# shayaanjamil-10xe/aimet

Measured on AMD Instinct MI355X. Metric: fake-quant Gelem/s (ResNet-50 W8A8 QuantSim forward QDQ; + compute_encodings wall-clock), higher is better.
Workload: dtype f32; 1 GPU; resnet50_w8a8_per_channel_fake_quant_fwd; launch=hipgraph, weight_qdq=one batched launch, global_batch=256, per_gpu_batch=256, act_quantizers=55, weight_quantizers=54, weight_channels=27560, parallelism=dp1, compute_encodings_scheme=tf_enhanced act per-tensor + tf_enhanced weight per-channel sym

## Files before the change

### aimet_amd/csrc/calib_plan.cpp

```cpp
#include <algorithm>
#include <cstring>
#include <mutex>
#include <vector>

#include "tq_internal.hpp"

using namespace aimet_amd;

struct aimet_calib_plan
{
    int device = 0;
    std::vector<aimet_tensor_quantizer*> aq, pq;
    int32_t aset[4] = {}, pset[4] = {};
    std::vector<StatsJob> jobs;
    uint64_t mm = 0, hb = 0;
    StatsJob* dj_fresh = nullptr;
    StatsJob* dj_cont  = nullptr;
    bool all_pdf       = false;
    ZeroJob* dz_act  = nullptr;
    int nz_act       = 0;
    int64_t most_act = 0;
    ResetJob* dr_act = nullptr;
    ZeroJob* dz_par  = nullptr;
    int nz_par       = 0;
    int64_t most_par = 0;
    ResetJob* dr_par = nullptr;
    ChannelJob* dch   = nullptr;
    uint64_t ch_blocks = 0;
    bool ch_hist      = false;
    TfeTable tfe_act {}, tfe_par {};
    bool has_tfe_act = false, has_tfe_par = false;
    void* pinned_act = nullptr;
    void* pinned_par = nullptr;
    size_t pinned_act_bytes = 0, pinned_par_bytes = 0;
    int busy_act = 0, busy_par = 0;
    void* dev_block = nullptr;
    hipEvent_t done = nullptr;
};

namespace
{

constexpr int kParamSearchPerCu = 2;

struct Packer
{
    std::vector<unsigned char> host;
    size_t add(const void* p, size_t bytes)
    {
        const size_t off = (host.size() + 255) & ~size_t(255);
        host.resize(off + bytes);
        if (bytes && p)
            std::memcpy(host.data() + off, p, bytes);
        return off;
    }
};

bool tfe_searched(const aimet_tensor_quantizer* q)
{
    return q->hist && q->scheme == AIMET_QUANTIZATION_TF_ENHANCED;
}

std::vector<TfeJob> tfe_jobs(const std::vector<aimet_tensor_quantizer*>& qs, int64_t* total)
{
    std::vector<TfeJob> jobs;
    int64_t t = 0;
    for (aimet_tensor_quantizer* q: qs)
        if (tfe_searched(q))
        {
            jobs.push_back(TfeJob {q->d.pdf_init, q->d.hist_min, q->d.bucket_size, q->d.pdf, nullptr, t});
            t += q->C;
        }
    *total = t;
    return jobs;
}

struct DeadPlan
{
    int device;
    void* dev_block;
    void* pinned_act;
    void* pinned_par;
    hipEvent_t done;
};
struct Graveyard
{
    std::mutex m;
    std::vector<DeadPlan> items;
};
Graveyard& graveyard()
{
    static Graveyard* g = new Graveyard();
    return *g;
}

void reap_dead_plans()
{
    std::vector<DeadPlan> ready;
    {
        Graveyard& g = graveyard();
        std::lock_guard<std::mutex> lock(g.m);
        for (size_t i = 0; i < g.items.size();)
            if (g.items[i].done == nullptr || hipEventQuery(g.items[i].done) == hipSuccess)
            {
                ready.push_back(g.items[i]);
// ... 10 lines not shown
        if (d.pinned_act)
            (void) hipHostFree(d.pinned_act);
        if (d.pinned_par)
            (void) hipHostFree(d.pinned_par);
        if (d.done)
            (void) hipEventDestroy(d.done);
    }
}

void destroy_plan(aimet_calib_plan* p)
{
    if (p == nullptr)
        return;
    if (p->dev_block || p->pinned_act || p->pinned_par || p->done)
    {
        Graveyard& g = graveyard();
        std::lock_guard<std::mutex> lock(g.m);
        g.items.push_back(DeadPlan {p->device, p->dev_block, p->pinned_act, p->pinned_par, p->done});
    }
    delete p;
}

hipStream_t upload_stream(int device)
{
    static std::mutex m;
    static std::vector<hipStream_t> streams(64, nullptr);
    AIMET_REQUIRE(device >= 0 && device < 64, "device id out of range");
    std::lock_guard<std::mutex> lock(m);
    if (streams[(size_t) device] == nullptr)
        AIMET_HIP_CHECK(hipStreamCreateWithFlags(&streams[(size_t) device], hipStreamNonBlocking));
    return streams[(size_t) device];
}

void adopt(aimet_encoding_request* r, void* pinned, size_t bytes, bool has_tfe, int* busy)
{
    if (r == nullptr)
        return;
    if (has_tfe)
    {
        r->pinned          = pinned;
        r->pinned_bytes    = bytes;
        r->pinned_borrowed = true;
    }
    r->busy = busy;
    ++*busy;
}

}

extern "C" {

int aimet_calib_plan_create(aimet_tensor_quantizer* const* act_qs, const float* const* act_x, const int64_t* act_n,
                            int64_t n_act, aimet_tensor_quantizer* const* par_qs, const float* const* par_x,
                            const int64_t* par_outer, const int64_t* par_C, const int64_t* par_K, int64_t n_par,
                            const int32_t* act_settings, const int32_t* par_settings, int64_t* elem_counts_dev,
                            aimet_calib_plan** out)
{
    aimet_calib_plan* p = nullptr;
    const int rc        = guarded([&] {
        AIMET_REQUIRE(out != nullptr && act_settings != nullptr && par_settings != nullptr, "null argument");
        AIMET_REQUIRE(n_act >= 0 && n_par >= 0, "negative quantizer count");
        AIMET_REQUIRE((n_act == 0 || (act_qs && act_x && act_n)) &&
                          (n_par == 0 || (par_qs && par_x && par_outer && par_C && par_K)),
                      "null argument");
        *out = nullptr;
        reap_dead_plans();
        p    = new aimet_calib_plan;
        std::copy(act_settings, act_settings + 4, p->aset);
        std::copy(par_settings, par_settings + 4, p->pset);
        p->aq.assign(act_qs, act_qs + n_act);
        p->pq.assign(par_qs, par_qs + n_par);
        AIMET_REQUIRE((n_act == 0 || act_qs[0] != nullptr) && (n_par == 0 || par_qs[0] != nullptr), "null quantizer");
        p->device = n_act ? act_qs[0]->device : (n_par ? par_qs[0]->device : 0);
        for (auto* q: p->pq)
            AIMET_REQUIRE(q != nullptr && q->device == p->device, "quantizers of one calibration share a device");
        if (elem_counts_dev)
            require_device_ptr(elem_counts_dev, "element counts");
        Packer pk;
        size_t o_fresh = 0, o_cont = 0, o_parts = 0, o_zact = 0, o_ract = 0;
        std::vector<int64_t> part_offs;
        if (n_act)
        {
            p->jobs = make_jobs(act_qs, act_x, act_n, nullptr, n_act);
            int64_t k = 0;
            p->all_pdf = true;
            for (int64_t i = 0; i < n_act; ++i)
            {
                StatsJob& j = p->jobs[(size_t) i];
                p->all_pdf  = p->all_pdf && j.hist && !j.ent;
                if (elem_counts_dev && j.hist)
                {
                    j.count_dev = elem_counts_dev + k;
                    j.count_out = elem_counts_dev + k;
                    ++k;
                }
            }
            stats_layout(p->jobs, &p->mm, &p->hb);
            o_parts = pk.add(nullptr, sizeof(float) * 2 * p->mm);
            std::vector<StatsJob> fresh = p->jobs;
            for (auto& j: fresh)
            {
                j.fresh = 1;
                j.seen  = 0;
            }
            for (auto& j: p->jobs)
                j.fresh = 0;
            o_fresh = pk.add(fresh.data(), sizeof(StatsJob) * fresh.size());
            o_cont  = pk.add(p->jobs.data(), sizeof(StatsJob) * p->jobs.size());
            std::vector<ZeroJob> z;
            std::vector<ResetJob> r;
            for (auto* q: p->aq)
                reset_ranges(q, false, z, r);
            for (const ZeroJob& zj: z)
                p->most_act = std::max(p->most_act, zj.bytes);
            p->nz_act = (int) z.size();
            o_zact    = pk.add(z.data(), sizeof(ZeroJob) * z.size());
            o_ract    = pk.add(r.data(), sizeof(ResetJob) * r.size());
        }
        size_t o_zpar = 0, o_rpar = 0, o_ch = 0;
        if (n_par)
        {
            std::vector<ChannelJob> cj;
            for (int64_t i = 0; i < n_par; ++i)
                cj.push_back(make_channel_job(par_qs[i], par_x[i], par_outer[i], par_C[i], par_K[i]));
            p->ch_blocks = channel_layout(cj, &p->ch_hist);
            o_ch         = pk.add(cj.data(), sizeof(ChannelJob) * cj.size());
            std::vector<ZeroJob> z;
            std::vector<ResetJob> r;
            for (auto* q: p->pq)
                reset_ranges(q, true, z, r);
            for (const ZeroJob& zj: z)
                p->most_par = std::max(p->most_par, zj.bytes);
            p->nz_par = (int) z.size();
            o_zpar    = pk.add(z.data(), sizeof(ZeroJob) * z.size());
            o_rpar    = pk.add(r.data(), sizeof(ResetJob) * r.size());
        }
        int64_t ta = 0, tp = 0;
        std::vector<TfeJob> ja = tfe_jobs(p->aq, &ta), jp = tfe_jobs(p->pq, &tp);
        DeviceGuard g(p->device);
        if (ta)
        {
            p->pinned_act_bytes = sizeof(aimet_tf_encoding) * (size_t) ta;
            AIMET_HIP_CHECK(hipHostMalloc(&p->pinned_act, p->pinned_act_bytes, hipHostMallocDefault));
            std::memset(p->pinned_act, 0, p->pinned_act_bytes);
        }
        if (tp)
        {
            p->pinned_par_bytes = sizeof(aimet_tf_encoding) * (size_t) tp;
            AIMET_HIP_CHECK(hipHostMalloc(&p->pinned_par, p->pinned_par_bytes, hipHostMallocDefault));
            std::memset(p->pinned_par, 0, p->pinned_par_bytes);
        }
        for (auto& j: ja)
            j.out = static_cast<aimet_tf_encoding*>(p->pinned_act) + j.start;
        for (auto& j: jp)
            j.out = static_cast<aimet_tf_encoding*>(p->pinned_par) + j.start;
        const int sa = ta ? tfe_splits(ta, p->aset[1] != 0) : 1, sp = tp ? tfe_splits(tp, p->pset[1] != 0) : 1;
        const size_t o_ja = pk.add(ja.data(), sizeof(TfeJob) * ja.size());
        const size_t o_jp = pk.add(jp.data(), sizeof(TfeJob) * jp.size());
        const size_t o_pa = sa > 1 ? pk.add(nullptr, sizeof(uint64_t) * 2 * ta * sa) : 0;
        const size_t o_ka = sa > 1 ? pk.add(nullptr, sizeof(unsigned) * ta) : 0;
        const size_t o_pp = sp > 1 ? pk.add(nullptr, sizeof(uint64_t) * 2 * tp * sp) : 0;
        const size_t o_kp = sp > 1 ? pk.add(nullptr, sizeof(unsigned) * tp) : 0;
        pk.add(nullptr, 0);
        if (pk.host.empty())
        {
            *out = p;
            p    = nullptr;
            return;
        }
        AIMET_HIP_CHECK(hipMalloc(&p->dev_block, pk.host.size()));
        char* base = static_cast<char*>(p->dev_block);
// ... 21 lines not shown
            p->dr_par = reinterpret_cast<ResetJob*>(base + o_rpar);
        }
        hipStream_t up = upload_stream(p->device);
        AIMET_HIP_CHECK(hipMemcpyAsync(p->dev_block, pk.host.data(), pk.host.size(), hipMemcpyHostToDevice, up));
        AIMET_HIP_CHECK(hipStreamSynchronize(up));
        AIMET_HIP_CHECK(hipEventCreateWithFlags(&p->done, hipEventDisableTiming));
        if (ta)
        {
            p->has_tfe_act = true;
            p->tfe_act     = TfeTable {ja[0], reinterpret_cast<const TfeJob*>(base + o_ja), (int) ja.size(), ta,
                                   sa > 1 ? reinterpret_cast<uint64_t*>(base + o_pa) : nullptr,
                                   sa > 1 ? reinterpret_cast<unsigned*>(base + o_ka) : nullptr};
        }
        if (tp)
        {
            p->has_tfe_par = true;
            p->tfe_par     = TfeTable {jp[0], reinterpret_cast<const TfeJob*>(base + o_jp), (int) jp.size(), tp,
                                   sp > 1 ? reinterpret_cast<uint64_t*>(base + o_pp) : nullptr,
                                   sp > 1 ? reinterpret_cast<unsigned*>(base + o_kp) : nullptr,
                                   n_act ? kParamSearchPerCu : 0};
        }
        *out = p;
        p    = nullptr;
    });
    if (p)
        destroy_plan(p);
    return rc;
}

int aimet_calib_plan_launch(aimet_calib_plan* p, int stages, int reset, void* main_stream, void* side_stream,
                            aimet_encoding_request** act_req, aimet_encoding_request** par_req)
{
    aimet_encoding_request *ra = nullptr, *rp = nullptr;
    const int rc = guarded([&] {
        AIMET_REQUIRE(p != nullptr && act_req != nullptr && par_req != nullptr, "null argument");
        AIMET_REQUIRE(stages >= 1 && stages <= 7 && (stages == 7 || stages == 1 || stages == 2 || stages == 4),
                      "stages: 7 (the whole batch on one device) or 1, 2, 4 (the sharded calibration's steps)");
        *act_req = *par_req = nullptr;
        const int64_t n_act = (int64_t) p->aq.size(), n_par = (int64_t) p->pq.size();
        if (n_act == 0 && n_par == 0)
            return;
        if ((stages & 4) && p->has_tfe_act)
            AIMET_REQUIRE(p->busy_act == 0, "calibration plan: the previous activation request is not finished");
        if ((stages & 1) && p->has_tfe_par)
            AIMET_REQUIRE(p->busy_par == 0, "calibration plan: the previous parameter request is not finished");
        DeviceGuard g(p->device);
        hipStream_t ms = as_stream(main_stream), ss = as_stream(side_stream);
        const bool first = (stages & 1) != 0;
        if (first && ss != ms && (n_par || (reset && n_act)))
            stream_join(ss, ms);
        auto rest = [&] {
            if (reset && n_act)
            {
                launch_zero_table(p->dz_act, p->nz_act, p->most_act, ss);
                launch_reset_table(p->dr_act, (int) n_act, ss);
                for (auto* q: p->aq)
                    mark_reset(q);
                if (ss != ms)
                    stream_join(ms, ss);
            }
            if (n_par)
            {
                if (reset)
                {
                    launch_zero_table(p->dz_par, p->nz_par, p->most_par, ss);
                    launch_reset_table(p->dr_par, (int) n_par, ss);
                    for (auto* q: p->pq)
                        mark_reset(q);
                }
                launch_channel_table(p->dch, (int) n_par, p->ch_blocks, p->ch_hist, ss);
                for (auto* q: p->pq)
                    q->stats_updated = true;
                encodings_launch(p->pq.data(), n_par, (uint32_t) p->pset[0], p->pset[1], p->pset[2], p->pset[3], ss, rp,
                                 nullptr, p->has_tfe_par ? &p->tfe_par : nullptr);
                adopt(rp, p->pinned_par, p->pinned_par_bytes, p->has_tfe_par, &p->busy_par);
            }
        };
        if (n_act)
        {
            int phases = 0;
            if (stages & 1)
                phases |= kPhaseMinmax | (stages == 7 ? kPhaseFoldMinmax : 0);
            if (stages & 2)
                phases |= (stages == 7 ? 0 : kPhaseFoldMinmax) | kPhaseHistogram;
            if (stages & 4)
                phases |= kPhaseFoldHistogram;
            bool seen = !reset;
            for (auto* q: p->aq)
                seen = seen && q->stats_updated;
            const bool walk = n_act > 64 || (p->all_pdf && seen);
            const StatsJob* dj = (first && reset) ? p->dj_fresh : p->dj_cont;
            if (first)
                launch_stats_table(dj, (int) n_act, p->mm, p->hb, walk, phases, ms, rest);
            else
                launch_stats_table(dj, (int) n_act, p->mm, p->hb, walk, phases, ms);
            if (first)
                for (auto* q: p->aq)
                    q->stats_updated = true;
        }
        else if (first)
            rest();
        if (stages & 4)
        {
            encodings_launch(p->aq.data(), n_act, (uint32_t) p->aset[0], p->aset[1], p->aset[2], p->aset[3], ms, ra,
                             nullptr, p->has_tfe_act ? &p->tfe_act : nullptr);
            adopt(ra, p->pinned_act, p->pinned_act_bytes, p->has_tfe_act, &p->busy_act);
        }
        if (first && n_par && ss != ms)
            stream_join(ms, ss);
        if (p->done)
            AIMET_HIP_CHECK(hipEventRecord(p->done, ms));
    });
    if (rc != AIMET_OK)
    {
        release_request_after_error(ra);
        release_request_after_error(rp);
        return rc;
    }
    *act_req = ra;
    *par_req = rp;
    return rc;
}

int aimet_calib_plan_destroy(aimet_calib_plan* p)
{
    return guarded([&] {
        if (p == nullptr)
            return;
        AIMET_REQUIRE(p->busy_act == 0 && p->busy_par == 0,
                      "calibration plan: finish (or discard) its requests before destroying it");
        destroy_plan(p);
    });
}

}
```

### aimet_amd/csrc/quantizer.cpp

```cpp
#include <algorithm>
#include <atomic>
#include <chrono>
#include <cstring>
#include <mutex>
#include <thread>
#include <vector>

#include "encodings.hpp"
#include "tq_internal.hpp"

using namespace aimet_amd;

struct Slab
{
    void* base   = nullptr;
    size_t bytes = 0;
    std::atomic<int64_t> refs {0};
};

namespace
{

size_t align256(size_t b)
{
// ... 956 lines not shown
    int64_t ent_total = 0;
    for (int64_t c: entC)
        ent_total += c;
    aimet_tf_encoding* mse_dst = nullptr;
    EntropyOut* ent_dst        = nullptr;
    if (req->mse_total + ent_total > 0)
    {
        const size_t mse_bytes = sizeof(aimet_tf_encoding) * (size_t) req->mse_total;
        req->pinned_dev = take_pinned(mse_bytes + sizeof(EntropyOut) * (size_t) ent_total, &req->pinned_dev_bytes);
        mse_dst         = req->mse_total ? static_cast<aimet_tf_encoding*>(req->pinned_dev) : nullptr;
        ent_dst = ent_total ? reinterpret_cast<EntropyOut*>(static_cast<char*>(req->pinned_dev) + mse_bytes) : nullptr;
    }
    launch_mse_search_many(mse.data(), mseC.data(), (int) mse.size(), b, sym != 0, strict != 0, unsign != 0, st,
                           mse_dst);
    launch_entropy_search_many(ent.data(), entC.data(), (int) ent.size(), sym != 0, strict != 0, unsign != 0, st,
                               ent_dst, b);
    if (tfe_total > 0 && table != nullptr)
    {
        AIMET_REQUIRE(table->total == tfe_total && table->n == (int) tfe.size(),
                      "calibration plan: the TF-Enhanced search table does not match the quantizers");
        launch_tfe_table(*table, b, sym != 0, strict != 0, unsign != 0, st);
    }
    else if (tfe_total > 0)
    {
        req->pinned = take_pinned(sizeof(aimet_tf_encoding) * (size_t) tfe_total, &req->pinned_bytes);
        launch_tfe_search_many_to(tfe.data(), req->tfe_Cs.data(), (int) tfe.size(), b, sym, strict, unsign,
                                  static_cast<aimet_tf_encoding*>(req->pinned), st, prep);
    }
    req->done = take_event();
    AIMET_HIP_CHECK(hipEventRecord(req->done, st));
    return req;
}

void aimet_amd::await_event(hipEvent_t e)
{
    const auto t0 = std::chrono::steady_clock::now();
    for (;;)
    {
        const hipError_t q = hipEventQuery(e);
        if (q == hipSuccess)
            return;
        if (q != hipErrorNotReady)
            AIMET_HIP_CHECK(q);
        const auto waited = std::chrono::steady_clock::now() - t0;
        if (waited > std::chrono::milliseconds(20))
            break;
        if (waited > std::chrono::microseconds(200))
            std::this_thread::sleep_for(std::chrono::microseconds(20));
    }
    AIMET_HIP_CHECK(hipEventSynchronize(e));
}

void aimet_amd::stream_join(hipStream_t waiter, hipStream_t from)
{
    hipEvent_t e = take_event();
    RequestPool& p = request_pool();
    try
    {
        AIMET_HIP_CHECK(hipEventRecord(e, from));
        AIMET_HIP_CHECK(hipStreamWaitEvent(waiter, e, 0));
    }
    catch (...)
    {
        std::lock_guard<std::mutex> lock(p.m);
        p.events.push_back(e);
        throw;
    }
    std::lock_guard<std::mutex> lock(p.m);
    p.events.push_back(e);
}

extern "C" {

int aimet_tq_get_encodings_launch(aimet_tensor_quantizer* const* qs, int64_t nq, uint32_t bw, int sym, int strict,
                                  int unsign, void* stream, aimet_encoding_request** req_out)
{
    aimet_encoding_request* req = nullptr;
    const int rc = guarded([&] {
        AIMET_REQUIRE(req_out != nullptr, "null argument");
        *req_out = nullptr;
        encodings_launch(qs, nq, bw, sym, strict, unsign, as_stream(stream), req);
    });
    if (rc != AIMET_OK)
// ... 70 lines not shown
        return rc;
    }
    *act_req = ra;
    *par_req = rp;
    return rc;
}

int aimet_tq_get_encodings_finish(aimet_encoding_request* req, aimet_tf_encoding* out, int* valid)
{
    const int rc = guarded([&] {
        AIMET_REQUIRE(req != nullptr, "request is null");
        const int64_t nq = (int64_t) req->qs.size();
        if (out == nullptr && valid == nullptr)
        {
            if (nq && req->done)
            {
                DeviceGuard g(req->device);
                AIMET_HIP_CHECK(hipEventSynchronize(req->done));
            }
            return;
        }
        int64_t total = 0;
        for (aimet_tensor_quantizer* q: req->qs)
            total += q->C;
        AIMET_REQUIRE(out != nullptr || total == 0, "out is null");
        if (total)
            std::memset(out, 0, sizeof(aimet_tf_encoding) * total);
        for (int64_t i = 0; i < nq; ++i)
            if (valid)
                valid[i] = req->qs[i]->stats_updated ? 1 : 0;
        if (nq == 0)
            return;
        DeviceGuard g(req->device);
        await_event(req->done);
        auto* tfe = static_cast<const aimet_tf_encoding*>(req->pinned);
        for (size_t k = 0, src = 0; k < req->tfe_Cs.size(); src += req->tfe_Cs[k], ++k)
            std::memcpy(out + req->tfe_offs[k], tfe + src, sizeof(aimet_tf_encoding) * req->tfe_Cs[k]);
        std::vector<int64_t> offs((size_t) nq);
        for (int64_t i = 0, o = 0; i < nq; o += req->qs[(size_t) i]->C, ++i)
            offs[(size_t) i] = o;
        std::vector<char> from_pinned((size_t) nq, 0);
        std::vector<const EntropyOut*> dev((size_t) nq, nullptr);
        {
            auto* m = static_cast<const aimet_tf_encoding*>(req->pinned_dev);
            for (int64_t i: req->mse_q)
            {
                const int64_t C = req->qs[(size_t) i]->C;
                std::memcpy(out + offs[(size_t) i], m, sizeof(aimet_tf_encoding) * C);
                m += C;
                from_pinned[(size_t) i] = 1;
            }
            auto* r = reinterpret_cast<const EntropyOut*>(static_cast<const char*>(req->pinned_dev) +
                                                          sizeof(aimet_tf_encoding) * (size_t) req->mse_total);
            for (int64_t i: req->ent_q)
            {
                const int64_t C = req->qs[(size_t) i]->C;
                aimet_tf_encoding* o = out + offs[(size_t) i];
                bool flagged = false;
                for (int64_t c = 0; c < C; ++c)
                {
                    o[c]    = aimet_tf_encoding {r[c].min, r[c].max, r[c].delta, r[c].offset, r[c].bw};
                    flagged = flagged || r[c].status == kEntHost;
                }
                dev[(size_t) i]         = r;
                from_pinned[(size_t) i] = flagged ? 0 : 1;
                r += C;
            }
// ... 105 lines not shown
```

### aimet_amd/csrc/stats.hip

```cpp
#include "entropy_core.hpp"
#include "tq_state.hpp"

#include <algorithm>
#include <cfloat>
#include <cstdlib>
#include <vector>

namespace aimet_amd
{

namespace
{

constexpr int kWaves      = kBlock / 64;
constexpr int kHistUnroll = 4;
constexpr int kHistGrid   = 2048;

__device__ __forceinline__ float wave_min(float v)
{
#pragma unroll
    for (int o = 32; o > 0; o >>= 1)
        v = fminf(v, __shfl_xor(v, o, 64));
    return v;
}
// ... 697 lines not shown
    }
}

__global__ __launch_bounds__(kBlock) void fold_minmax_many_kernel(const StatsJob* __restrict__ jobs)
{
    const StatsJob& J = jobs[blockIdx.x];
    if (J.ent)
    {
        float2 m = reinterpret_cast<const float2*>(J.d.minmax)[0];
        ent_fold_one(J.d, 0, -m.x, m.y);
    }
    else if (threadIdx.x == 0)
        fold_one(J.d, 0, !J.hist);
}

template <int BLOCK, int COLS>
__global__ __launch_bounds__(BLOCK) void histogram_many_kernel(const StatsJob* __restrict__ jobs, int njobs)
{
    const StatsJob& J = jobs[find_job(jobs, njobs, blockIdx.x, true)];
    if (!J.hist)
        return;
    if (J.ent)
    {
        if (J.d.active[0])
            histogram_part<BLOCK, true, COLS>(J.x, J.n, J.vec, blockIdx.x - J.h_block0, J.h_blocks, J.d);
    }
    else if (J.d.pdf_init[0])
        histogram_part<BLOCK, false, COLS>(J.x, J.n, J.vec, blockIdx.x - J.h_block0, J.h_blocks, J.d);
}

__global__ __launch_bounds__(kPdfSize) void fold_histogram_many_kernel(const StatsJob* __restrict__ jobs)
{
    const StatsJob& J = jobs[blockIdx.x];
    if (!J.hist)
        return;
    if (J.ent)
    {
        if (J.d.active[0])
            ent_fold_hist_one(J.d, 0);
    }
    else if (J.d.pdf_init[0])
        fold_hist_one(J.d, 0, J.count_dev ? *J.count_dev : J.count);
}

__device__ __forceinline__ int find_channel_job(const ChannelJob* __restrict__ jobs, int njobs, uint32_t b)
{
    return find_job_ballot(jobs, njobs, b, [](const ChannelJob& j) { return j.block0; });
}

__device__ __forceinline__ void channel_minmax(const ChannelJob& J, int64_t c, float& mn, float& mx)
{
    mn = INFINITY;
    mx = -INFINITY;
    for (int64_t o = 0; o < J.outer; ++o)
    {
        const float* row = J.x + (o * J.C + c) * J.K;
        if (J.vec)
        {
            const float4* r4 = reinterpret_cast<const float4*>(row);
            for (int64_t k = threadIdx.x; k < J.K / 4; k += kBlock)
                accum4(r4[k], mn, mx);
        }
        else
        {
            for (int64_t k = threadIdx.x; k < J.K; k += kBlock)
            {
                mn = fminf(mn, row[k]);
// ... 410 lines not shown
```

### aimet_amd/csrc/tfe_core.hpp

```cpp
#pragma once

#include <cfloat>
#include <cmath>

#if defined(__HIPCC__)
#define AIMET_HD __host__ __device__
#else
#define AIMET_HD
#endif

namespace aimet_amd
{
namespace tfe
{

constexpr int kBins        = 512;
constexpr float kGamma     = 3.0f;
constexpr float kMinRangeF = (float) 0.01;
constexpr int kAsymF       = 17;
constexpr int kAsymO       = 21;
constexpr int kSymF        = 101;
constexpr int kMaxCand     = kAsymF * kAsymO + 1;

template <class T>
// ... 301 lines not shown
    if constexpr (!split)
    {
        for (int k = 0; k < B.nnz; ++k)
        {
            if (k < kLo)
            {
                double d = B.cd_c[k] - loMid;
                satLo += B.pdf_c[k] * (d * d);
            }
            if (k >= kHi)
            {
                double d = B.cd_c[k] - hiMid;
                satHi += B.pdf_c[k] * (d * d);
            }
            if (k >= kLo && k < kHi)
            {
                float v   = B.cf_c[k];
                int q     = quant_code(v, delta, offset, rcp, thr);
                float deq = delta * (q + offset);
                double d  = (double) (v - deq);
                quant += B.pdf_c[k] * (d * d);
            }
        }
        double c = kGamma * (satLo + satHi) + quant;
        return smin(c, DBL_MAX);
    }
    satLo = sat_sum(B, 0, kLo, loMid);
    satHi = sat_sum(B, kHi, B.nnz, hiMid);
    quant = quant_sum(B, kLo, kHi, delta, offset, rcp, thr);
    double c = kGamma * (satLo + satHi) + quant;
    return smin(c, DBL_MAX);
}

struct Result
{
    double min, max, delta, offset;
};

AIMET_HD inline Result finish(const Setup& s, float bestDelta, int bestOffset)
{
    float lo = smax(bestDelta * bestOffset, -FLT_MAX);
    float hi = smin(bestDelta * (bestOffset + s.steps), FLT_MAX);
    return Result {lo, hi, bestDelta, (double) bestOffset};
}

}
}
```

### aimet_amd/csrc/tfe_search.hip

```cpp
#include "tfe_core.hpp"

#include <algorithm>
#include <cstdlib>
#include <cstring>
#include <mutex>
#include "tq_state.hpp"

#include <mutex>
#include <vector>

namespace aimet_amd
{
namespace
{

struct Best
{
    double cost;
    int idx;
    float delta;
    int offset;
};

__device__ __forceinline__ bool better(const Best& a, const Best& b)
{
    if (a.idx < 0)
        return false;
    if (b.idx < 0)
        return true;
    return (a.cost < b.cost) || (a.cost == b.cost && a.idx < b.idx);
}

template <int BLOCK, bool SYMFORM>
__global__ __launch_bounds__(BLOCK, BLOCK == 128 ? 5 : (BLOCK == 64 ? 2 : 7)) void tfe_search_kernel(
    TfeJob one, const TfeJob* __restrict__ jobs, int njobs, int64_t total, int bw, int sym, int strict, int unsign,
    int splits, uint64_t* __restrict__ part, unsigned* __restrict__ tickets)
{
    constexpr int kW = BLOCK / 64;
    __shared__ double pdf_c[tfe::kBins];
    __shared__ double cd_c[tfe::kBins];
    __shared__ float cf_c[tfe::kBins];
    __shared__ float cf[tfe::kBins];
    __shared__ short pos[tfe::kBins];
    __shared__ float fseq[tfe::kSymF + 8];
    __shared__ int first, last, nnz;
    __shared__ Best wbest[kW];
    if (threadIdx.x == 0)
    {
        if (sym)
            tfe::fseq_sym(fseq);
        else
            tfe::fseq_asym(fseq);
    }
    const int lane = threadIdx.x & 63;
    for (int64_t gs = blockIdx.x; gs < total * splits; gs += gridDim.x)
    {
        const int64_t g = gs / splits;
        const int sp    = (int) (gs - g * splits);
        TfeJob j = one;
        if (jobs)
        {
            int lo = 0, hi = njobs - 1;
            while (lo < hi)
            {
                int mid = (lo + hi + 1) >> 1;
                if (jobs[mid].start <= g)
                    lo = mid;
                else
                    hi = mid - 1;
            }
            j = jobs[lo];
        }
        const int64_t c = g - j.start;
        if (!j.pdf_init[c])
        {
            if (threadIdx.x == 0 && sp == 0)
            {
                int isteps = (int) (float) (ldexp(1.0, bw) - 1);
                aimet_tf_encoding e;
                e.delta    = (1.0 - (-1.0)) / isteps;
                e.offset   = floor(-1.0 / e.delta);
                e.min      = e.offset * e.delta;
                e.max      = e.min + isteps * e.delta;
                e.bw       = bw;
                j.out[c]   = e;
            }
            continue;
        }
        tfe::Hist h {j.hist_min[c], j.bucket_size[c], nullptr};
        const float start = tfe::bins_start(h);
        const double step = tfe::bins_step(h);
        for (int i = threadIdx.x; i < tfe::kBins; i += BLOCK)
            pdf_c[i] = j.pdf[c * tfe::kBins + i];
        __syncthreads();
        if (threadIdx.x < 64)
        {
            const bool skip = tfe::bins_skip_empty(h);
            const unsigned long long below = (1ull << lane) - 1;
            int base = 0, fst = -1, lst = -1;
            for (int i0 = 0; i0 < tfe::kBins; i0 += 64)
            {
                const int i          = i0 + lane;
                const double pi      = pdf_c[i];
                const double m_c     = tfe::bin_centre(start, step, i);
                const bool occupied  = pi > 0;
                const bool visit     = occupied || !skip;
                unsigned long long m = __ballot(visit);
                unsigned long long o = __ballot(occupied);
                const int k          = base + __popcll(m & below);
                cf[i]                = (float) m_c;
                pos[i]               = (short) k;
                if (visit)
                {
                    pdf_c[k] = pi;
                    cd_c[k]  = m_c;
                    cf_c[k]  = (float) m_c;
                }
                base += __popcll(m);
                if (o)
                {
                    if (fst < 0)
                        fst = i0 + __ffsll((long long) o) - 1;
                    lst = i0 + 63 - __clzll(o);
                }
            }
            if (lane == 0)
            {
                nnz   = base;
                first = fst;
                last  = lst > 0 ? lst : -1;
            }
        }
        __syncthreads();
        float lo, hi;
        tfe::observed_range(h, first, last, lo, hi);
        tfe::Setup st = tfe::setup(lo, hi, bw, sym != 0, strict != 0, unsign != 0);
        const tfe::Bins B {start, step, cf, pdf_c, cd_c, cf_c, pos, nnz};

        Best b {0.0, -1, -1.0f, -1};
        for (int t = threadIdx.x + sp * BLOCK; t < st.ncand; t += BLOCK * splits)
        {
            float dl;
            int o;
            if (!tfe::candidate(st, fseq, t, dl, o))
                continue;
            double cst = tfe::cost<SYMFORM>(B, bw, dl, o);
            if (!(cst < DBL_MAX))
                continue;
            Best me {cst, t, dl, o};
            if (better(me, b))
                b = me;
        }
        for (int k = 32; k > 0; k >>= 1)
        {
            Best o;
            o.cost   = __shfl_xor(b.cost, k, 64);
            o.idx    = __shfl_xor(b.idx, k, 64);
            o.delta  = __shfl_xor(b.delta, k, 64);
            o.offset = __shfl_xor(b.offset, k, 64);
            if (better(o, b))
                b = o;
        }
        if (lane == 0)
            wbest[threadIdx.x >> 6] = b;
        __syncthreads();
        if (threadIdx.x == 0)
            for (int w = 1; w < kW; ++w)
                if (better(wbest[w], b))
                    b = wbest[w];
        bool finish = splits == 1;
        if (!finish)
        {
            __shared__ int lastw;
            if (threadIdx.x == 0)
            {
                uint64_t* my = part + 2 * gs;
                publish_u64(my, (uint64_t) __double_as_longlong(b.cost));
                publish_u64(my + 1, (uint64_t) (uint32_t) b.idx);
                lastw = arrive_is_last(tickets + g, (unsigned) splits);
            }
            __syncthreads();
            if (lastw)
            {
                __builtin_amdgcn_fence(__ATOMIC_ACQUIRE, "wavefront");
                double qc = 0.0;
                int qi    = -1;
                if (threadIdx.x < (unsigned) splits)
                {
                    const uint64_t* pq = part + 2 * (g * splits + threadIdx.x);
                    qc                 = __longlong_as_double((long long) consume_u64(pq));
                    qi                 = (int) (uint32_t) consume_u64(pq + 1);
                }
                Best m {0.0, -1, -1.0f, -1};
                for (int q = 0; q < splits; ++q)
                {
                    Best o {__shfl(qc, q, 64), __shfl(qi, q, 64), -1.0f, -1};
                    if (better(o, m))
                        m = o;
                }
                if (threadIdx.x == 0)
                {
                    finish = true;
                    b      = m;
                    if (b.idx >= 0)
                        tfe::candidate(st, fseq, b.idx, b.delta, b.offset);
                    ticket_reset(tickets + g);
                }
            }
        }
        if (threadIdx.x == 0 && finish)
        {
            float bd = b.idx >= 0 ? b.delta : -1.0f;
            int bo   = b.idx >= 0 ? b.offset : -1;
            tfe::Result r = tfe::finish(st, bd, bo);
            j.out[c]      = aimet_tf_encoding {r.min, r.max, r.delta, r.offset, bw};
        }
        __syncthreads();
    }
}

constexpr int kSearchGridCap = 65536;

constexpr int64_t kTfeSplitBelow = 512;

void launch_split(const TfeJob& one, const TfeJob* jobs, int njobs, int64_t total, int bw, bool sym, bool strict,
                  bool unsign, int splits, uint64_t* part, unsigned* tickets, hipStream_t s)
{
    const int grid = (int) std::min<int64_t>(total * splits, kSearchGridCap);
    if (sym)
        tfe_search_kernel<64, true><<<grid, 64, 0, s>>>(one, jobs, njobs, total, bw, 1, strict, unsign, splits, part,
                                                      tickets);
    else
        tfe_search_kernel<64, false><<<grid, 64, 0, s>>>(one, jobs, njobs, total, bw, 0, strict, unsign, splits, part,
                                                       tickets);
    AIMET_LAUNCH_CHECK();
}

void launch_kernel(const TfeJob& one, const TfeJob* jobs, int njobs, int64_t total, int bw, bool sym, bool strict,
                   bool unsign, hipStream_t s, size_t lds_pad = 0)
{
    const int cap    = kSearchGridCap;
    const int splits = tfe_splits(total, sym);
    if (splits > 1)
    {
        unsigned* tickets = ticket_alloc(s, (unsigned) total);
        if (tickets)
        {
            auto* part = static_cast<uint64_t*>(scratch_alloc(sizeof(uint64_t) * 2 * total * splits, s));
            launch_split(one, jobs, njobs, total, bw, sym, strict, unsign, splits, part, tickets, s);
            scratch_free(part, s);
            return;
        }
    }
    const int grid = (int) (total < cap ? total : cap);
    if (sym)
        tfe_search_kernel<128, true><<<grid, 128, lds_pad, s>>>(one, jobs, njobs, total, bw, 1, strict, unsign, 1, nullptr,
                                                        nullptr);
    else
        tfe_search_kernel<384, false><<<grid, 384, lds_pad, s>>>(one, jobs, njobs, total, bw, 0, strict, unsign, 1, nullptr,
                                                         nullptr);
    AIMET_LAUNCH_CHECK();
}

}

int tfe_splits(int64_t total, bool sym)
{
// ... 119 lines not shown
```

### aimet_amd/csrc/tq_internal.hpp

```cpp
#pragma once

#include <vector>

#include "tq_state.hpp"

struct Slab;

struct aimet_tensor_quantizer
{
    int scheme       = AIMET_QUANTIZATION_TF;
    int64_t C        = 1;
    int device       = 0;
    float percentile = 100.0f;
    bool stats_updated = false;
    bool hist        = false;
    aimet_amd::StatsKind kind = aimet_amd::kKindTf;
    void* arena      = nullptr;
    size_t arena_bytes = 0;
    Slab* slab = nullptr;
    aimet_amd::TqDevice d {};
};

struct aimet_encoding_request
{
    std::vector<aimet_tensor_quantizer*> qs;
    int32_t b  = 0;
    int sym    = 0, strict = 0, unsign = 0;
    int device = 0;
    hipStream_t stream = nullptr;
    hipEvent_t done = nullptr;
    void* pinned    = nullptr;
    size_t pinned_bytes = 0;
    bool pinned_borrowed = false;
    int* busy = nullptr;
    std::vector<int64_t> tfe_offs, tfe_Cs;
    void* pinned_dev        = nullptr;
    size_t pinned_dev_bytes = 0;
    std::vector<int64_t> mse_q, ent_q;
    int64_t mse_total = 0;
};

namespace aimet_amd
{

struct DeviceGuard
{
    int prev = -1;
    explicit DeviceGuard(int dev)
    {
        AIMET_HIP_CHECK(hipGetDevice(&prev));
        if (prev != dev)
            AIMET_HIP_CHECK(hipSetDevice(dev));
    }
    ~DeviceGuard()
    {
        int cur = -1;
        if (hipGetDevice(&cur) == hipSuccess && cur != prev && prev >= 0)
            (void) hipSetDevice(prev);
    }
};

std::vector<StatsJob> make_jobs(aimet_tensor_quantizer* const* qs, const float* const* xs, const int64_t* ns,
                                const int64_t* counts, int64_t count, const int64_t* counts_dev = nullptr);
ChannelJob make_channel_job(aimet_tensor_quantizer* q, const float* x, int64_t outer, int64_t C, int64_t K);
void reset_ranges(const aimet_tensor_quantizer* q, bool light, std::vector<ZeroJob>& zero,
                  std::vector<ResetJob>& resets);
void mark_reset(aimet_tensor_quantizer* q);

bool device_search(const aimet_tensor_quantizer* q);
bool entropy_device(const aimet_tensor_quantizer* q, int32_t b);

void* take_pinned(size_t bytes, size_t* real);
hipEvent_t take_event();
void give_event(hipEvent_t e);
void release_request(aimet_encoding_request* r);
void await_event(hipEvent_t e);
void release_request_after_error(aimet_encoding_request* r);

aimet_encoding_request* encodings_launch(aimet_tensor_quantizer* const* qs, int64_t nq, uint32_t bw, int sym,
                                         int strict, int unsign, hipStream_t st, aimet_encoding_request*& req,
                                         hipStream_t prep = nullptr, const TfeTable* tfe = nullptr);

}
```

### aimet_amd/csrc/tq_state.hpp

```cpp
#pragma once

#include <cstddef>
#include <functional>

#include "common.hpp"

#include <vector>

namespace aimet_amd
{

struct TqDevice
{
    float* minmax;
    float* partials;
    double* acc;
    int32_t* pdf_init;
    int32_t* iterations;
    float* hist_min;
    double* bucket_size;
    float* bin_bucket;
    float* bin_offset;
    double* pdf;
    unsigned long long* counts;
// ... 17 lines not shown
void launch_fold_minmax(const TqDevice& d, int64_t C, StatsKind kind, hipStream_t s);
void launch_batch_histogram(const TqDevice& d, const float* x, int64_t outer, int64_t C, int64_t K, StatsKind kind,
                            hipStream_t s);
void launch_fold_histogram(const TqDevice& d, int64_t C, int64_t count, StatsKind kind, hipStream_t s);
void launch_reset_state(const TqDevice& d, int64_t C, bool hist, hipStream_t s);
struct ResetJob
{
    double* acc;
    int64_t C;
};
void launch_reset_state_many(const std::vector<ResetJob>& jobs, hipStream_t s);
struct ZeroJob
{
    void* p;
    int64_t bytes;
};
void launch_zero_many(const std::vector<ZeroJob>& jobs, hipStream_t s);
void launch_zero_table(const ZeroJob* dj, int n, int64_t most, hipStream_t s);
void launch_reset_table(const ResetJob* dj, int n, hipStream_t s);
struct StatsJob
{
    const float* x;
    int64_t n;
    int64_t count;
    const int64_t* count_dev;
    int64_t* count_out;
    TqDevice d;
    uint32_t mm_block0, mm_blocks, h_block0, h_blocks;
    float* mm_part;
    int32_t hist, vec;
    int32_t ent;
    int32_t seen;
    int32_t fresh;
};
enum StatsPhase
{
    kPhaseMinmax        = 1,
    kPhaseFoldMinmax    = 2,
    kPhaseHistogram     = 4,
    kPhaseFoldHistogram = 8
};
void launch_stats_many(std::vector<StatsJob>& jobs, int phases, hipStream_t s,
                       const std::function<void()>& between = {});
void stats_layout(std::vector<StatsJob>& jobs, uint64_t* mm, uint64_t* hb);
bool stats_walk(const StatsJob* jobs, int n);
void launch_stats_table(const StatsJob* dj, int n, uint64_t mm, uint64_t hb, bool walk, int phases, hipStream_t s,
                        const std::function<void()>& between = {});
struct ChannelJob
{
    const float* x;
    int64_t outer, C, K;
    TqDevice d;
    uint32_t block0;
    int32_t kind;
    int32_t vec;
};
void launch_channel_stats_many(std::vector<ChannelJob>& jobs, hipStream_t s);
uint64_t channel_layout(std::vector<ChannelJob>& jobs, bool* any_hist);
void launch_channel_table(const ChannelJob* dj, int n, uint64_t blocks, bool any_hist, hipStream_t s);
struct TfeJob
{
    const int32_t* pdf_init;
    const float* hist_min;
    const double* bucket_size;
    const double* pdf;
    aimet_tf_encoding* out;
    int64_t start;
};
struct TfeTable
{
    TfeJob first {};
    const TfeJob* dev = nullptr;
    int n = 0;
    int64_t total = 0;
    uint64_t* part = nullptr;
    unsigned* tickets = nullptr;
    int per_cu = 0;
};
int tfe_splits(int64_t total, bool sym);
void launch_tfe_table(const TfeTable& t, int bw, bool sym, bool strict, bool unsign, hipStream_t s);
void launch_tfe_search(const TqDevice& d, int64_t C, int bw, bool sym, bool strict, bool unsign, hipStream_t s);
void launch_tfe_search_many(const TqDevice* const* ds, const int64_t* Cs, int n, int bw, bool sym, bool strict,
                            bool unsign, aimet_tf_encoding* host_out, hipStream_t s);
void launch_tfe_search_many_to(const TqDevice* const* ds, const int64_t* Cs, int n, int bw, bool sym, bool strict,
                               bool unsign, aimet_tf_encoding* pinned_dst, hipStream_t s, hipStream_t prep = nullptr);
void stream_join(hipStream_t waiter, hipStream_t from);
size_t mse_part_bytes(int64_t C);
void launch_mse_search(const TqDevice& d, int64_t C, int bw, bool sym, bool strict, bool unsign, hipStream_t s);
void launch_mse_search_many(const TqDevice* const* ds, const int64_t* Cs, int n, int bw, bool sym, bool strict,
                            bool unsign, hipStream_t s, aimet_tf_encoding* pinned_dst = nullptr);

enum EntropyStatus
{
    kEntFinal  = 0,
    kEntHost   = 1,
    kEntNoHist = 2
};
struct EntropyRange
{
    float lo, hi;
// ... 21 lines not shown
```

Before: 829.6 Gelem/s.

## Fuse histogram fold into TFE search, spread cost sums across waves, adaptive host wait

```diff
diff --git a/aimet_amd/csrc/calib_plan.cpp b/aimet_amd/csrc/calib_plan.cpp
--- a/aimet_amd/csrc/calib_plan.cpp
+++ b/aimet_amd/csrc/calib_plan.cpp
@@ -17,6 +17,7 @@
     StatsJob* dj_fresh = nullptr;
     StatsJob* dj_cont  = nullptr;
     bool all_pdf       = false;
+    bool fold_launch   = false;
     ZeroJob* dz_act  = nullptr;
     int nz_act       = 0;
     int64_t most_act = 0;
@@ -34,6 +35,7 @@
     void* pinned_par = nullptr;
     size_t pinned_act_bytes = 0, pinned_par_bytes = 0;
     int busy_act = 0, busy_par = 0;
+    int64_t span_act_ns = 0, span_par_ns = 0;
     void* dev_block = nullptr;
     hipEvent_t done = nullptr;
 };
@@ -61,16 +63,28 @@
     return q->hist && q->scheme == AIMET_QUANTIZATION_TF_ENHANCED;
 }
 
-std::vector<TfeJob> tfe_jobs(const std::vector<aimet_tensor_quantizer*>& qs, int64_t* total)
+std::vector<TfeJob> tfe_jobs(const std::vector<aimet_tensor_quantizer*>& qs, int64_t* total,
+                             const std::vector<StatsJob>* stats = nullptr)
 {
     std::vector<TfeJob> jobs;
     int64_t t = 0;
-    for (aimet_tensor_quantizer* q: qs)
-        if (tfe_searched(q))
-        {
-            jobs.push_back(TfeJob {q->d.pdf_init, q->d.hist_min, q->d.bucket_size, q->d.pdf, nullptr, t});
-            t += q->C;
-        }
+    for (size_t i = 0; i < qs.size(); ++i)
+    {
+        aimet_tensor_quantizer* q = qs[i];
+        if (!tfe_searched(q))
+            continue;
+        TfeJob j {q->d.pdf_init, q->d.hist_min, q->d.bucket_size, q->d.pdf, nullptr, t};
+        if (stats && (*stats)[i].fold_in_search)
+        {
+            j.counts     = q->d.counts;
+            j.pdf_rw     = q->d.pdf;
+            j.iterations = q->d.iterations;
+            j.count_dev  = (*stats)[i].count_dev;
+            j.count      = (*stats)[i].count;
+        }
+        jobs.push_back(j);
+        t += q->C;
+    }
     *total = t;
     return jobs;
 }
@@ -147,10 +161,13 @@
     return streams[(size_t) device];
 }
 
-void adopt(aimet_encoding_request* r, void* pinned, size_t bytes, bool has_tfe, int* busy)
+void adopt(aimet_encoding_request* r, void* pinned, size_t bytes, bool has_tfe, int* busy, int64_t* span_ns,
+           std::chrono::steady_clock::time_point entered)
 {
     if (r == nullptr)
         return;
+    r->launched = entered;
+    r->span_ns  = span_ns;
     if (has_tfe)
     {
         r->pinned          = pinned;
@@ -210,6 +227,16 @@
                     ++k;
                 }
             }
+            int64_t searched = 0;
+            for (int64_t i = 0; i < n_act; ++i)
+                searched += tfe_searched(act_qs[i]) ? 1 : 0;
+            const bool split = searched > 0 && tfe_splits(searched, p->aset[1] != 0) > 1;
+            for (int64_t i = 0; i < n_act; ++i)
+            {
+                StatsJob& j      = p->jobs[(size_t) i];
+                j.fold_in_search = split && tfe_searched(act_qs[i]) ? 1 : 0;
+                p->fold_launch   = p->fold_launch || (j.hist && !j.fold_in_search);
+            }
             stats_layout(p->jobs, &p->mm, &p->hb);
             o_parts = pk.add(nullptr, sizeof(float) * 2 * p->mm);
             std::vector<StatsJob> fresh = p->jobs;
@@ -251,7 +278,7 @@
             o_rpar    = pk.add(r.data(), sizeof(ResetJob) * r.size());
         }
         int64_t ta = 0, tp = 0;
-        std::vector<TfeJob> ja = tfe_jobs(p->aq, &ta), jp = tfe_jobs(p->pq, &tp);
+        std::vector<TfeJob> ja = tfe_jobs(p->aq, &ta, &p->jobs), jp = tfe_jobs(p->pq, &tp);
         DeviceGuard g(p->device);
         if (ta)
         {
@@ -339,6 +366,7 @@
                             aimet_encoding_request** act_req, aimet_encoding_request** par_req)
 {
     aimet_encoding_request *ra = nullptr, *rp = nullptr;
+    const auto entered = std::chrono::steady_clock::now();
     const int rc = guarded([&] {
         AIMET_REQUIRE(p != nullptr && act_req != nullptr && par_req != nullptr, "null argument");
         AIMET_REQUIRE(stages >= 1 && stages <= 7 && (stages == 7 || stages == 1 || stages == 2 || stages == 4),
@@ -354,9 +382,19 @@
         DeviceGuard g(p->device);
         hipStream_t ms = as_stream(main_stream), ss = as_stream(side_stream);
         const bool first = (stages & 1) != 0;
+        struct Fork
+        {
+            hipEvent_t e = nullptr;
+            ~Fork() { give_event(e); }
+        } fork;
         if (first && ss != ms && (n_par || (reset && n_act)))
-            stream_join(ss, ms);
+        {
+            fork.e = take_event();
+            AIMET_HIP_CHECK(hipEventRecord(fork.e, ms));
+        }
         auto rest = [&] {
+            if (fork.e)
+                AIMET_HIP_CHECK(hipStreamWaitEvent(ss, fork.e, 0));
             if (reset && n_act)
             {
                 launch_zero_table(p->dz_act, p->nz_act, p->most_act, ss);
@@ -380,7 +418,8 @@
                     q->stats_updated = true;
                 encodings_launch(p->pq.data(), n_par, (uint32_t) p->pset[0], p->pset[1], p->pset[2], p->pset[3], ss, rp,
                                  nullptr, p->has_tfe_par ? &p->tfe_par : nullptr);
-                adopt(rp, p->pinned_par, p->pinned_par_bytes, p->has_tfe_par, &p->busy_par);
+                adopt(rp, p->pinned_par, p->pinned_par_bytes, p->has_tfe_par, &p->busy_par, &p->span_par_ns,
+                      entered);
             }
         };
         if (n_act)
@@ -390,7 +429,7 @@
                 phases |= kPhaseMinmax | (stages == 7 ? kPhaseFoldMinmax : 0);
             if (stages & 2)
                 phases |= (stages == 7 ? 0 : kPhaseFoldMinmax) | kPhaseHistogram;
-            if (stages & 4)
+            if ((stages & 4) && p->fold_launch)
                 phases |= kPhaseFoldHistogram;
             bool seen = !reset;
             for (auto* q: p->aq)
@@ -411,7 +450,8 @@
         {
             encodings_launch(p->aq.data(), n_act, (uint32_t) p->aset[0], p->aset[1], p->aset[2], p->aset[3], ms, ra,
                              nullptr, p->has_tfe_act ? &p->tfe_act : nullptr);
-            adopt(ra, p->pinned_act, p->pinned_act_bytes, p->has_tfe_act, &p->busy_act);
+            adopt(ra, p->pinned_act, p->pinned_act_bytes, p->has_tfe_act, &p->busy_act, &p->span_act_ns,
+                  entered);
         }
         if (first && n_par && ss != ms)
             stream_join(ms, ss);
diff --git a/aimet_amd/csrc/quantizer.cpp b/aimet_amd/csrc/quantizer.cpp
--- a/aimet_amd/csrc/quantizer.cpp
+++ b/aimet_amd/csrc/quantizer.cpp
@@ -1012,23 +1012,56 @@
     return req;
 }
 
-void aimet_amd::await_event(hipEvent_t e)
-{
-    const auto t0 = std::chrono::steady_clock::now();
-    for (;;)
-    {
+void aimet_amd::await_event(hipEvent_t e, std::chrono::steady_clock::time_point launched, int64_t* span_ns)
+{
+    using clock = std::chrono::steady_clock;
+    using std::chrono::duration_cast;
+    using std::chrono::nanoseconds;
+    constexpr int64_t kSpanMargin = 100 * 1000;
+    constexpr int64_t kSleepStep  = 200 * 1000;
+    constexpr auto kSpin          = std::chrono::microseconds(200);
+    const auto t0 = clock::now();
+    clock::time_point busy_at {};
+    bool saw_busy = false;
+    auto finished = [&]() -> bool {
         const hipError_t q = hipEventQuery(e);
+        if (q != hipSuccess && q != hipErrorNotReady)
+            AIMET_HIP_CHECK(q);
         if (q == hipSuccess)
+        {
+            if (span_ns != nullptr && saw_busy)
+                *span_ns = std::max<int64_t>(1, duration_cast<nanoseconds>(busy_at - launched).count());
+            return true;
+        }
+        saw_busy = true;
+        busy_at  = clock::now();
+        return false;
+    };
+    if (finished())
+        return;
+    const int64_t record = span_ns != nullptr ? *span_ns : 0;
+    while (record > 0)
+    {
+        const int64_t left = record - kSpanMargin - duration_cast<nanoseconds>(clock::now() - launched).count();
+        if (left <= 0)
+            break;
+        std::this_thread::sleep_for(nanoseconds(std::min(left, kSleepStep)));
+        if (finished())
             return;
-        if (q != hipErrorNotReady)
-            AIMET_HIP_CHECK(q);
-        const auto waited = std::chrono::steady_clock::now() - t0;
-        if (waited > std::chrono::milliseconds(20))
-            break;
-        if (waited > std::chrono::microseconds(200))
-            std::this_thread::sleep_for(std::chrono::microseconds(20));
+    }
+    const auto spin0 = clock::now();
+    while (clock::now() - spin0 < kSpin)
+        if (finished())
+            return;
+    while (clock::now() - t0 < std::chrono::milliseconds(20))
+    {
+        std::this_thread::sleep_for(std::chrono::microseconds(20));
+        if (finished())
+            return;
     }
     AIMET_HIP_CHECK(hipEventSynchronize(e));
+    if (span_ns != nullptr && saw_busy)
+        *span_ns = std::max<int64_t>(1, duration_cast<nanoseconds>(busy_at - launched).count());
 }
 
 void aimet_amd::stream_join(hipStream_t waiter, hipStream_t from)
@@ -1165,7 +1198,7 @@
         if (nq == 0)
             return;
         DeviceGuard g(req->device);
-        await_event(req->done);
+        await_event(req->done, req->launched, req->span_ns);
         auto* tfe = static_cast<const aimet_tf_encoding*>(req->pinned);
         for (size_t k = 0, src = 0; k < req->tfe_Cs.size(); src += req->tfe_Cs[k], ++k)
             std::memcpy(out + req->tfe_offs[k], tfe + src, sizeof(aimet_tf_encoding) * req->tfe_Cs[k]);
diff --git a/aimet_amd/csrc/stats.hip b/aimet_amd/csrc/stats.hip
--- a/aimet_amd/csrc/stats.hip
+++ b/aimet_amd/csrc/stats.hip
@@ -753,7 +753,7 @@
 __global__ __launch_bounds__(kPdfSize) void fold_histogram_many_kernel(const StatsJob* __restrict__ jobs)
 {
     const StatsJob& J = jobs[blockIdx.x];
-    if (!J.hist)
+    if (!J.hist || J.fold_in_search)
         return;
     if (J.ent)
     {
diff --git a/aimet_amd/csrc/tfe_core.hpp b/aimet_amd/csrc/tfe_core.hpp
--- a/aimet_amd/csrc/tfe_core.hpp
+++ b/aimet_amd/csrc/tfe_core.hpp
@@ -357,6 +357,35 @@
     return smin(c, DBL_MAX);
 }
 
+AIMET_HD inline double cost_sum(const Bins& B, int bw, float delta, int offset, int which)
+{
+    const float lo    = delta * offset;
+    const float steps = (float) (ldexp(1.0, bw) - 1);
+    const float hi    = delta * (offset + steps);
+    int iLo           = (int) floor((lo - B.start) / B.step);
+    iLo               = smin(smax(0, iLo), kBins - 1);
+    int iHi           = (int) floor((hi - B.start) / B.step);
+    iHi               = smin(smax(0, iHi), kBins - 1);
+    const float loMid = B.cf[iLo];
+    const float hiMid = B.cf[iHi];
+    const int kLo     = B.pos[iLo];
+    const int kHi     = B.pos[iHi];
+    if (which == 1)
+        return sat_sum(B, 0, kLo, loMid);
+    if (which == 2)
+        return sat_sum(B, kHi, B.nnz, hiMid);
+    const float rcp  = 1.0f / delta;
+    const float vmax = (loMid != loMid || hiMid != hiMid) ? NAN : smax(fabsf(loMid), fabsf(hiMid));
+    const float thr  = (vmax * rcp + fabsf((float) offset) + 1.0f) * 4.76837158203125e-7f;
+    return quant_sum(B, kLo, kHi, delta, offset, rcp, thr);
+}
+
+AIMET_HD inline double cost_total(double satLo, double satHi, double quant)
+{
+    double c = kGamma * (satLo + satHi) + quant;
+    return smin(c, DBL_MAX);
+}
+
 struct Result
 {
     double min, max, delta, offset;
diff --git a/aimet_amd/csrc/tfe_search.hip b/aimet_amd/csrc/tfe_search.hip
--- a/aimet_amd/csrc/tfe_search.hip
+++ b/aimet_amd/csrc/tfe_search.hip
@@ -31,8 +31,8 @@
     return (a.cost < b.cost) || (a.cost == b.cost && a.idx < b.idx);
 }
 
-template <int BLOCK, bool SYMFORM>
-__global__ __launch_bounds__(BLOCK, BLOCK == 128 ? 5 : (BLOCK == 64 ? 2 : 7)) void tfe_search_kernel(
+template <int BLOCK, bool SYMFORM, bool SPREAD = false>
+__global__ __launch_bounds__(BLOCK, BLOCK == 128 ? 5 : (SPREAD ? 2 : 7)) void tfe_search_kernel(
     TfeJob one, const TfeJob* __restrict__ jobs, int njobs, int64_t total, int bw, int sym, int strict, int unsign,
     int splits, uint64_t* __restrict__ part, unsigned* __restrict__ tickets)
 {
@@ -43,8 +43,9 @@
     __shared__ float cf[tfe::kBins];
     __shared__ short pos[tfe::kBins];
     __shared__ float fseq[tfe::kSymF + 8];
-    __shared__ int first, last, nnz;
+    __shared__ int first, last, nnz, fin;
     __shared__ Best wbest[kW];
+    static_assert(!SPREAD || BLOCK == 192, "three waves, one per sum of the cost");
     if (threadIdx.x == 0)
     {
         if (sym)
@@ -90,8 +91,15 @@
         tfe::Hist h {j.hist_min[c], j.bucket_size[c], nullptr};
         const float start = tfe::bins_start(h);
         const double step = tfe::bins_step(h);
+        const bool fold        = SPREAD && j.counts != nullptr;
+        const int fold_it      = fold ? j.iterations[c] : 0;
+        const double fold_n    = fold ? (double) (j.count_dev ? *j.count_dev : j.count) : 0.0;
+        auto folded            = [&](int i) {
+            const double prob = (double) j.counts[c * tfe::kBins + i] / fold_n;
+            return fold_it == 0 ? prob : (j.pdf_rw[c * tfe::kBins + i] * fold_it + prob) / (fold_it + 1);
+        };
         for (int i = threadIdx.x; i < tfe::kBins; i += BLOCK)
-            pdf_c[i] = j.pdf[c * tfe::kBins + i];
+            pdf_c[i] = fold ? folded(i) : j.pdf[c * tfe::kBins + i];
         __syncthreads();
         if (threadIdx.x < 64)
         {
@@ -138,19 +146,44 @@
         const tfe::Bins B {start, step, cf, pdf_c, cd_c, cf_c, pos, nnz};
 
         Best b {0.0, -1, -1.0f, -1};
-        for (int t = threadIdx.x + sp * BLOCK; t < st.ncand; t += BLOCK * splits)
-        {
-            float dl;
-            int o;
-            if (!tfe::candidate(st, fseq, t, dl, o))
-                continue;
-            double cst = tfe::cost<SYMFORM>(B, bw, dl, o);
-            if (!(cst < DBL_MAX))
-                continue;
-            Best me {cst, t, dl, o};
-            if (better(me, b))
-                b = me;
-        }
+        if constexpr (SPREAD)
+        {
+            __shared__ double sat[2][64];
+            const int which = threadIdx.x >> 6;
+            for (int t0 = sp * 64; t0 < st.ncand; t0 += 64 * splits)
+            {
+                const int t = t0 + lane;
+                float dl    = 0.0f;
+                int o       = 0;
+                const bool ok = t < st.ncand && tfe::candidate(st, fseq, t, dl, o);
+                const double sum = ok ? tfe::cost_sum(B, bw, dl, o, which) : 0.0;
+                if (which)
+                    sat[which - 1][lane] = sum;
+                __syncthreads();
+                if (which == 0 && ok)
+                {
+                    const double cst = tfe::cost_total(sat[0][lane], sat[1][lane], sum);
+                    const Best me {cst, t, dl, o};
+                    if (cst < DBL_MAX && better(me, b))
+                        b = me;
+                }
+                __syncthreads();
+            }
+        }
+        else
+            for (int t = threadIdx.x + sp * BLOCK; t < st.ncand; t += BLOCK * splits)
+            {
+                float dl;
+                int o;
+                if (!tfe::candidate(st, fseq, t, dl, o))
+                    continue;
+                double cst = tfe::cost<SYMFORM>(B, bw, dl, o);
+                if (!(cst < DBL_MAX))
+                    continue;
+                Best me {cst, t, dl, o};
+                if (better(me, b))
+                    b = me;
+            }
         for (int k = 32; k > 0; k >>= 1)
         {
             Best o;
@@ -215,6 +248,20 @@
             tfe::Result r = tfe::finish(st, bd, bo);
             j.out[c]      = aimet_tf_encoding {r.min, r.max, r.delta, r.offset, bw};
         }
+        if (fold)
+        {
+            if (threadIdx.x == 0)
+                fin = finish;
+            __syncthreads();
+            if (fin)
+                for (int i = threadIdx.x; i < tfe::kBins; i += BLOCK)
+                {
+                    j.pdf_rw[c * tfe::kBins + i] = folded(i);
+                    j.counts[c * tfe::kBins + i] = 0;
+                }
+            if (threadIdx.x == 0 && finish)
+                j.iterations[c] = fold_it + 1;
+        }
         __syncthreads();
     }
 }
@@ -227,12 +274,8 @@
                   bool unsign, int splits, uint64_t* part, unsigned* tickets, hipStream_t s)
 {
     const int grid = (int) std::min<int64_t>(total * splits, kSearchGridCap);
-    if (sym)
-        tfe_search_kernel<64, true><<<grid, 64, 0, s>>>(one, jobs, njobs, total, bw, 1, strict, unsign, splits, part,
-                                                      tickets);
-    else
-        tfe_search_kernel<64, false><<<grid, 64, 0, s>>>(one, jobs, njobs, total, bw, 0, strict, unsign, splits, part,
-                                                       tickets);
+    tfe_search_kernel<192, false, true><<<grid, 192, 0, s>>>(one, jobs, njobs, total, bw, sym ? 1 : 0, strict, unsign,
+                                                             splits, part, tickets);
     AIMET_LAUNCH_CHECK();
 }
 
diff --git a/aimet_amd/csrc/tq_internal.hpp b/aimet_amd/csrc/tq_internal.hpp
--- a/aimet_amd/csrc/tq_internal.hpp
+++ b/aimet_amd/csrc/tq_internal.hpp
@@ -1,5 +1,6 @@
 #pragma once
 
+#include <chrono>
 #include <vector>
 
 #include "tq_state.hpp"
@@ -33,6 +34,8 @@
     size_t pinned_bytes = 0;
     bool pinned_borrowed = false;
     int* busy = nullptr;
+    std::chrono::steady_clock::time_point launched {};
+    int64_t* span_ns = nullptr;
     std::vector<int64_t> tfe_offs, tfe_Cs;
     void* pinned_dev        = nullptr;
     size_t pinned_dev_bytes = 0;
@@ -74,7 +77,7 @@
 hipEvent_t take_event();
 void give_event(hipEvent_t e);
 void release_request(aimet_encoding_request* r);
-void await_event(hipEvent_t e);
+void await_event(hipEvent_t e, std::chrono::steady_clock::time_point launched = {}, int64_t* span_ns = nullptr);
 void release_request_after_error(aimet_encoding_request* r);
 
 aimet_encoding_request* encodings_launch(aimet_tensor_quantizer* const* qs, int64_t nq, uint32_t bw, int sym,
diff --git a/aimet_amd/csrc/tq_state.hpp b/aimet_amd/csrc/tq_state.hpp
--- a/aimet_amd/csrc/tq_state.hpp
+++ b/aimet_amd/csrc/tq_state.hpp
@@ -73,6 +73,7 @@
     int32_t ent;
     int32_t seen;
     int32_t fresh;
+    int32_t fold_in_search;
 };
 enum StatsPhase
 {
@@ -107,6 +108,11 @@
     const double* pdf;
     aimet_tf_encoding* out;
     int64_t start;
+    unsigned long long* counts;
+    double* pdf_rw;
+    int32_t* iterations;
+    const int64_t* count_dev;
+    int64_t count;
 };
 struct TfeTable
 {
```

New measurement: 828.0 Gelem/s. Within noise of the previous version (-0.2%).
